# pirovc/ganon

Measured on AMD Instinct MI355X. Metric: Mreads/s classified (150 bp) + IBF-lookup GB/s vs HBM roofline, higher is better.
Workload: dtype u64

## Files before the change

### ganon_amd/csrc/gn_minimiser_lpr.hip

```cpp
#include "gn_internal.h"
#include <type_traits>

#define GN_WAVE 64

namespace
{
struct LprRankLut
{
    uint8_t t[256];
    constexpr LprRankLut() : t{}
    {
        for (int i = 0; i < 256; ++i)
            t[i] = 0;
        t['C'] = t['c'] = 1;
        t['G'] = t['g'] = 2;
        t['T'] = t['t'] = t['U'] = t['u'] = 3;
        t['Y'] = t['y'] = 1;
        t['S'] = t['s'] = 1;
        t['K'] = t['k'] = 2;
        t['B'] = t['b'] = 1;
    }
};
}
__constant__ LprRankLut GN_LPR_RANK_LUT = LprRankLut();

__device__ __forceinline__ uint32_t gn_lpr_wave_max(uint32_t v)
{
#pragma unroll
    for (int off = 32; off >= 1; off >>= 1)
    {
        const uint32_t o = __shfl_xor(v, off);
        v                = o > v ? o : v;
    }
    return v;
}
__device__ __forceinline__ unsigned long long gn_lpr_wave_sum(unsigned long long v)
{
#pragma unroll
    for (int off = 32; off >= 1; off >>= 1)
        v += __shfl_xor(v, off);
    return v;
}

typedef uint32_t gn_u32x4u __attribute__((ext_vector_type(4), aligned(4)));

__global__ __launch_bounds__(64) void gn_minimiser_lpr_kernel(GnMinimiserParams p)
{
    extern __shared__ __attribute__((aligned(16))) uint8_t gn_lpr_smem[];
    const uint32_t lane = threadIdx.x;
    const uint32_t k = p.k, w = p.w;
    const uint32_t K = w - k + 1;
    uint64_t*      bufV = reinterpret_cast<uint64_t*>(gn_lpr_smem);
    uint8_t*       bufP = gn_lpr_smem + (size_t)2 * K * GN_WAVE * 8;
    const uint64_t seed = 0x8F3F73B5CF1C9ADEULL >> (64u - 2u * k);
    const uint64_t mask = k == 32 ? ~0ULL : ((1ULL << (2 * k)) - 1ULL);

    const uint32_t r   = p.read_begin + blockIdx.x * GN_WAVE + lane;
    const bool     inr = r < p.n_reads;
    uint64_t       b1 = 0, len1 = 0, b2 = 0, len2 = 0;
    if (inr)
    {
        b1   = p.off1[r];
        len1 = p.off1[r + 1] - b1;
        if (p.off2)
        {
            b2   = p.off2[r];
            len2 = p.off2[r + 1] - b2;
        }
    }
    const bool too_long = len1 > p.lpr_max_len || len2 > p.lpr_max_len;
    const bool mine     = inr && !too_long;
    if (inr && too_long)
        p.defer_list[atomicAdd(p.defer_count, 1ULL)] = r;

    uint8_t  st = GN_READ_OK;
    uint32_t n  = 0;
    if (mine && len1 < w)
        st = GN_READ_SMALL;
    uint64_t* out = p.hashes + (mine ? p.slot_off[r] : 0);

    for (uint32_t seg = 0; seg < 2; ++seg)
    {
        const uint64_t L64  = seg ? len2 : len1;
        const bool     act  = mine && st == GN_READ_OK && L64 >= w;
        const uint32_t Leff = act ? (uint32_t)L64 : 0u;
        const uint32_t Lmax = gn_lpr_wave_max(Leff);
        if (Lmax == 0)
            continue;
        const uintptr_t  sa  = reinterpret_cast<uintptr_t>(p.bases + (seg ? b2 : b1));
        const uint32_t   o   = (uint32_t)(sa & 3u);
        const uint32_t*  dws = reinterpret_cast<const uint32_t*>(sa & ~(uintptr_t)3);
        const uint32_t   ndw = Leff ? (o + Leff + 3) / 4 : 0;
        auto load4 = [&](uint32_t q) -> gn_u32x4u {
            const uint32_t qc = q < ndw ? q : (ndw ? ndw - 1 : 0u);
            return *reinterpret_cast<const gn_u32x4u*>(dws + qc);
        };
        gn_u32x4u cur4 = load4(0), nxt4 = load4(4);

        uint64_t f = 0, rc = 0;
        uint64_t pre_v = ~0ULL, Wprev = 0;
        uint32_t pre_p = 0, expiry = 0xFFFFFFFFu;
        uint32_t blk = 0, pin = 0;

        auto position = [&](uint32_t i, uint32_t c) {
            const bool on = i < Leff;
            uint64_t   v  = ~0ULL;
            if (on)
            {
                uint64_t       b      = ((c >> 1) ^ (c >> 2)) & 3u;
                const bool     simple = ((0x0030008Au >> (c & 31u)) & 1u) && (c & 0xC0u) == 0x40u;
                if (!simple)
                    b = GN_LPR_RANK_LUT.t[c];
                f                = ((f << 2) | b) & mask;
                rc               = (rc >> 2) | ((3ULL - b) << (2 * (k - 1)));
                const uint64_t x = f ^ seed, y = rc ^ seed;
                v                = x < y ? x : y;
            }
            if (i + 1 < k)
                return;
            const uint32_t pk = i + 1 - k;
            bufV[((size_t)blk * K + pin) * GN_WAVE + lane] = v;
            if (pin == 0 || v <= pre_v)
            {
                pre_v = v;
                pre_p = pk;
            }
            if (pk + 1 >= K)
            {
                const uint32_t j = pk + 1 - K;
                uint64_t       W = pre_v;
                uint32_t       R = pre_p;
                if (pin != K - 1)
                {
                    const size_t   s  = ((size_t)(blk ^ 1u) * K + (pin + 1)) * GN_WAVE + lane;
                    const uint64_t sv = bufV[s];
                    if (sv < pre_v)
                    {
                        W = sv;
                        R = (pk - pin - K) + bufP[s];
                    }
                }
                if (on)
                {
                    const bool emit = j == 0 || j == expiry || v < Wprev;
                    if (emit)
                    {
                        out[n++] = W;
                        expiry   = R + 1u;
                    }
                    Wprev = W;
                }
            }
            if (pin == K - 1)
            {
                uint64_t run_v = ~0ULL;
                uint32_t run_p = K - 1;
                for (int t = (int)K - 1; t >= 0; --t)
                {
                    const size_t   s = ((size_t)blk * K + (uint32_t)t) * GN_WAVE + lane;
                    const uint64_t x = bufV[s];
                    if (x < run_v || t == (int)K - 1)
                    {
                        run_v = x;
                        run_p = (uint32_t)t;
                    }
                    bufV[s] = run_v;
                    bufP[s] = (uint8_t)run_p;
                }
                blk ^= 1u;
                pin = 0;
            }
            else
                ++pin;
        };

        for (uint32_t i0 = 0; i0 < Lmax; i0 += 16)
        {
            const gn_u32x4u nn4 = load4(i0 / 4 + 8);
            uint32_t        d[8] = { cur4.x, cur4.y, cur4.z, cur4.w, nxt4.x, nxt4.y, nxt4.z, nxt4.w };
#pragma unroll
            for (int u = 0; u < 4; ++u)
            {
                const uint64_t win = ((uint64_t)d[u + 1] << 32) | d[u];
#pragma unroll
                for (int t = 0; t < 4; ++t)
                {
                    const uint32_t i = i0 + 4 * u + t;
                    if (i < Lmax)
                        position(i, (uint32_t)(win >> (8u * (o + t))) & 0xFFu);
                }
            }
            cur4 = nxt4;
            nxt4 = nn4;
        }
    }
    unsigned long long mine_total = 0;
    if (mine)
    {
        if (n > 65535u)
            st = GN_READ_BIG;
        else if (st == GN_READ_OK)
            mine_total = n;
        p.n_hashes[r] = n;
        p.status[r]   = st;
    }
    mine_total = gn_lpr_wave_sum(mine_total);
    if (lane == 0 && mine_total)
        atomicAdd(p.total_hashes + (blockIdx.x & 63u), mine_total);
}

#define GN_LPRK_STAGE 24u

template <bool FMIN>
__device__ __forceinline__ uint64_t gn_key_min(uint64_t a, uint64_t b)
{
    if constexpr (FMIN)
    {
        uint64_t r;
        asm("v_min_f64 %0, %1, %2" : "=v"(r) : "v"(a), "v"(b));
        return r;
    }
    else
        return a < b ? a : b;
}

template <int KW, bool FMIN>
__global__ __launch_bounds__(64) void gn_minimiser_lprk_kernel(GnMinimiserParams p)
{
    __shared__ uint64_t stage[GN_LPRK_STAGE * (GN_WAVE + 1)];
    const uint32_t lane = threadIdx.x;
    __shared__ uint8_t rank_lut[256];
#pragma unroll
    for (uint32_t t = 0; t < 4; ++t)
    {
        const uint32_t c   = lane * 4 + t, idx = c & 31u;
        uint32_t       b32 = ((0x0238000Cu >> idx) & 1u) | (((0x00300880u >> idx) & 1u) << 1);
        rank_lut[c]        = (uint8_t)((c & 0xC0u) == 0x40u ? b32 : 0u);
    }
    __builtin_amdgcn_fence(__ATOMIC_RELEASE, "wavefront");
    __builtin_amdgcn_wave_barrier();
    __builtin_amdgcn_fence(__ATOMIC_ACQUIRE, "wavefront");
    const uint32_t k    = p.k;
    const uint64_t seed = 0x8F3F73B5CF1C9ADEULL >> (64u - 2u * k);
    const uint64_t mask = (1ULL << (2 * k)) - 1ULL;
    const uint32_t w    = k + KW - 1;

    const uint32_t r   = p.read_begin + blockIdx.x * GN_WAVE + lane;
    const bool     inr = r < p.n_reads;
    uint64_t       b1 = 0, len1 = 0, b2 = 0, len2 = 0;
    if (inr)
    {
        b1   = p.off1[r];
        len1 = p.off1[r + 1] - b1;
        if (p.off2)
        {
            b2   = p.off2[r];
            len2 = p.off2[r + 1] - b2;
        }
    }
    const bool too_long = len1 > p.lpr_max_len || len2 > p.lpr_max_len;
    const bool mine     = inr && !too_long;
    if (inr && too_long)
        p.defer_list[atomicAdd(p.defer_count, 1ULL)] = r;

    uint8_t  st = GN_READ_OK;
    uint32_t n  = 0;
    if (mine && len1 < w)
        st = GN_READ_SMALL;
    const uint64_t out_base = mine ? p.slot_off[r] : 0;

    for (uint32_t seg = 0; seg < 2; ++seg)
    {
        const uint64_t L64  = seg ? len2 : len1;
        const bool     act  = mine && st == GN_READ_OK && L64 >= w;
        const uint32_t Leff = act ? (uint32_t)L64 : 0u;
        const uint32_t Lmax = gn_lpr_wave_max(Leff);
        if (Lmax == 0)
            continue;
        const uint32_t Lmin = ~gn_lpr_wave_max(~Leff);
        const uint32_t n_seg0 = n;
        const uintptr_t sa  = reinterpret_cast<uintptr_t>(p.bases + (seg ? b2 : b1));
        const uint32_t  o   = (uint32_t)(sa & 3u);
        const uint32_t* dws = reinterpret_cast<const uint32_t*>(sa & ~(uintptr_t)3);
        const uint32_t  ndw = Leff ? (o + Leff + 3) / 4 : 0;
        auto dword_at = [&](uint32_t q) -> uint32_t {
            const uint32_t qc = q < ndw ? q : (ndw ? ndw - 1 : 0u);
            return dws[qc];
        };

        uint64_t       f = 0, rcx = mask;
        const uint64_t seed_rc = seed ^ mask;
        const uint32_t top     = 2 * (k - 1);
        auto roll = [&](uint32_t c) -> uint64_t {
            const uint64_t b = rank_lut[c];
            f                  = ((f << 2) | b) & mask;
            rcx                = (rcx >> 2) | (b << top);
            const uint64_t x = f ^ seed, y = rcx ^ seed_rc;
            return gn_key_min<FMIN>(x, y);
        };
        for (uint32_t q = 0; q * 4 < o + k - 1; ++q)
        {
            const uint32_t dw = dword_at(q);
#pragma unroll
            for (uint32_t t = 0; t < 4; ++t)
            {
                const uint32_t by = q * 4 + t;
                if (by >= o && by - o + 1 < k)
                    (void)roll((dw >> (8u * t)) & 0xFFu);
            }
        }

        uint64_t V[KW], S[KW];
#pragma unroll
        for (int t = 0; t < KW; ++t)
            V[t] = S[t] = ~0ULL;
        uint64_t pre = ~0ULL, Wprev = 0;
        uint32_t expiry = 0xFFFFFFFFu;
        const uint32_t M = Lmax - k + 1;

        constexpr int NDW = (KW + 3) / 4 + 1;
        uint32_t      cur[NDW], nxt[NDW];
        auto fetch = [&](uint32_t blk, uint32_t* dst) {
            const uint32_t q = (o + k - 1 + blk * KW) >> 2;
#pragma unroll
            for (int d = 0; d < NDW; ++d)
                dst[d] = dword_at(q + d);
        };
        fetch(0, cur);
        for (uint32_t blk = 0; blk * KW < M; ++blk)
        {
            fetch(blk + 1, nxt);
            const uint32_t sh = (o + k - 1 + blk * KW) & 3u;
            uint32_t       by[NDW - 1];
#pragma unroll
            for (int d = 0; d + 1 < NDW; ++d)
                by[d] = __builtin_amdgcn_alignbyte(cur[d + 1], cur[d], sh);
            auto block = [&](auto all_on_tag) {
            constexpr bool ALL_ON = decltype(all_on_tag)::value;
#pragma unroll
            for (int pin = 0; pin < KW; ++pin)
            {
                const uint32_t pk = blk * KW + pin;
                const uint32_t i  = pk + k - 1;
                const bool     on = ALL_ON || i < Leff;
                const uint32_t c  = (by[pin >> 2] >> (8 * (pin & 3))) & 0xFFu;
                const uint64_t kv  = (roll(c) << 16) | (uint64_t)(0xFFFFu - pk);
                const uint64_t key = on ? kv : ~0ULL;
                V[pin] = key;
                pre    = pin == 0 ? key : gn_key_min<FMIN>(key, pre);
                if (pk + 1 >= KW)
                {
                    const uint32_t j = pk + 1 - KW;
                    uint64_t       W = pre;
                    if (pin != KW - 1)
                        W = gn_key_min<FMIN>(S[(pin + 1) % KW], pre);
                    if (on)
                    {
                        const bool emit = j == 0 || j == expiry || (key | 0xFFFFull) < (Wprev & ~0xFFFFull);
                        if (emit)
                        {
                            const uint32_t e = n - n_seg0;
                            if (e < GN_LPRK_STAGE)
                                stage[e * (GN_WAVE + 1) + lane] = W >> 16;
                            else
                                p.hashes[out_base + n] = W >> 16;
                            ++n;
                            expiry = (0xFFFFu - (uint32_t)(W & 0xFFFFu)) + 1u;
                        }
                        Wprev = W;
                    }
                }
            }
            };
            if ((blk + 1) * KW + k - 1 <= Lmin)
                block(std::true_type{});
            else
                block(std::false_type{});
            S[KW - 1] = V[KW - 1];
#pragma unroll
            for (int t = KW - 2; t >= 0; --t)
                S[t] = gn_key_min<FMIN>(V[t], S[t + 1]);
#pragma unroll
            for (int d = 0; d < NDW; ++d)
                cur[d] = nxt[d];
        }
        __builtin_amdgcn_fence(__ATOMIC_RELEASE, "wavefront");
        __builtin_amdgcn_wave_barrier();
        __builtin_amdgcn_fence(__ATOMIC_ACQUIRE, "wavefront");
        const uint32_t cnt_mine = act ? (n - n_seg0 < GN_LPRK_STAGE ? n - n_seg0 : GN_LPRK_STAGE) : 0u;
        uint64_t       todo     = __ballot(cnt_mine != 0);
        while (todo)
        {
            const int l = __builtin_ctzll(todo);
            todo &= todo - 1;
            const uint32_t cnt = (uint32_t)__builtin_amdgcn_readlane((int)cnt_mine, l);
            const uint64_t dst0 = out_base + n_seg0;
            const uint64_t dst  = ((uint64_t)(uint32_t)__builtin_amdgcn_readlane((int)(dst0 >> 32), l) << 32) |
                                 (uint32_t)__builtin_amdgcn_readlane((int)(uint32_t)dst0, l);
            if (lane < cnt)
                p.hashes[dst + lane] = stage[lane * (GN_WAVE + 1) + (uint32_t)l];
        }
        __builtin_amdgcn_fence(__ATOMIC_RELEASE, "wavefront");
        __builtin_amdgcn_wave_barrier();
        __builtin_amdgcn_fence(__ATOMIC_ACQUIRE, "wavefront");
    }
    unsigned long long mine_total = 0;
    if (mine)
    {
        if (n > 65535u)
            st = GN_READ_BIG;
        else if (st == GN_READ_OK)
            mine_total = n;
        p.n_hashes[r] = n;
        p.status[r]   = st;
    }
    mine_total = gn_lpr_wave_sum(mine_total);
    if (lane == 0 && mine_total)
        atomicAdd(p.total_hashes + (blockIdx.x & 63u), mine_total);
}

template <int KW>
static void gn_launch_lprk(const GnMinimiserParams& p, hipStream_t st)
{
    const dim3 grid((p.n_reads - p.read_begin + GN_WAVE - 1) / GN_WAVE);
    if (p.k <= 20)
        hipLaunchKernelGGL((gn_minimiser_lprk_kernel<KW, true>), grid, dim3(GN_WAVE), 0, st, p);
    else
        hipLaunchKernelGGL((gn_minimiser_lprk_kernel<KW, false>), grid, dim3(GN_WAVE), 0, st, p);
}

hipError_t gn_launch_minimiser_lpr(const GnMinimiserParams& p, hipStream_t st)
{
    if (p.n_reads <= p.read_begin)
        return hipSuccess;
    const uint32_t K   = p.w - p.k + 1;
    if (K <= 16 && p.k <= 24)
    {
        switch (K)
        {
            case 1: gn_launch_lprk<1>(p, st); break;
            case 2: gn_launch_lprk<2>(p, st); break;
            case 3: gn_launch_lprk<3>(p, st); break;
            case 4: gn_launch_lprk<4>(p, st); break;
            case 5: gn_launch_lprk<5>(p, st); break;
            case 6: gn_launch_lprk<6>(p, st); break;
            case 7: gn_launch_lprk<7>(p, st); break;
            case 8: gn_launch_lprk<8>(p, st); break;
            case 9: gn_launch_lprk<9>(p, st); break;
            case 10: gn_launch_lprk<10>(p, st); break;
            case 11: gn_launch_lprk<11>(p, st); break;
            case 12: gn_launch_lprk<12>(p, st); break;
            case 13: gn_launch_lprk<13>(p, st); break;
            case 14: gn_launch_lprk<14>(p, st); break;
            case 15: gn_launch_lprk<15>(p, st); break;
            default: gn_launch_lprk<16>(p, st); break;
        }
        return hipGetLastError();
    }
    const size_t   lds = (size_t)2 * K * GN_WAVE * 9;
    (void)hipFuncSetAttribute(reinterpret_cast<const void*>(gn_minimiser_lpr_kernel), hipFuncAttributeMaxDynamicSharedMemorySize,
                              (int)lds);
    hipLaunchKernelGGL(gn_minimiser_lpr_kernel, dim3((p.n_reads - p.read_begin + GN_WAVE - 1) / GN_WAVE), dim3(GN_WAVE), lds, st, p);
    return hipGetLastError();
}
```

Baseline: 271.3.

## Split LPR minimiser rolling hash into 32-bit halves and make emission branchless

Rewrites the per-read minimiser kernel so the rolling k-mer state is kept as 32-bit halves, with a 32-bit-only path when k<=16 under FMIN. Emission becomes branchless: every step writes unconditionally into a split 32/16-bit LDS stage, and overflow is handled through a ballot-guarded global store. The kernel also sets waves_per_eu, peels the first block, prefetches ranks in an interleaved way, and flushes two lanes per trip. These changes aim to cut 64-bit ALU work, divergence and register pressure. The cost is extra LDS writes per step and more complex code.

```diff
diff --git a/ganon_amd/csrc/gn_minimiser_lpr.hip b/ganon_amd/csrc/gn_minimiser_lpr.hip
--- a/ganon_amd/csrc/gn_minimiser_lpr.hip
+++ b/ganon_amd/csrc/gn_minimiser_lpr.hip
@@ -210,6 +210,7 @@
 }
 
 #define GN_LPRK_STAGE 24u
+#define GN_LPRK_ROW (GN_WAVE + 1u)
 
 template <bool FMIN>
 __device__ __forceinline__ uint64_t gn_key_min(uint64_t a, uint64_t b)
@@ -224,10 +225,13 @@
         return a < b ? a : b;
 }
 
+__device__ __forceinline__ uint64_t gn_u64_of(uint32_t hi, uint32_t lo) { return ((uint64_t)hi << 32) | lo; }
+
 template <int KW, bool FMIN>
-__global__ __launch_bounds__(64) void gn_minimiser_lprk_kernel(GnMinimiserParams p)
-{
-    __shared__ uint64_t stage[GN_LPRK_STAGE * (GN_WAVE + 1)];
+__global__ __launch_bounds__(64) __attribute__((amdgpu_waves_per_eu(KW <= 13 ? 4 : 3))) void gn_minimiser_lprk_kernel(GnMinimiserParams p)
+{
+    __shared__ uint32_t stage_lo[(GN_LPRK_STAGE + 1u) * GN_LPRK_ROW];
+    __shared__ uint16_t stage_hi[(GN_LPRK_STAGE + 1u) * GN_LPRK_ROW];
     const uint32_t lane = threadIdx.x;
     __shared__ uint8_t rank_lut[256];
 #pragma unroll
@@ -247,16 +251,12 @@
 
     const uint32_t r   = p.read_begin + blockIdx.x * GN_WAVE + lane;
     const bool     inr = r < p.n_reads;
-    uint64_t       b1 = 0, len1 = 0, b2 = 0, len2 = 0;
+    uint64_t       len1 = 0, len2 = 0;
     if (inr)
     {
-        b1   = p.off1[r];
-        len1 = p.off1[r + 1] - b1;
+        len1 = p.off1[r + 1] - p.off1[r];
         if (p.off2)
-        {
-            b2   = p.off2[r];
-            len2 = p.off2[r + 1] - b2;
-        }
+            len2 = p.off2[r + 1] - p.off2[r];
     }
     const bool too_long = len1 > p.lpr_max_len || len2 > p.lpr_max_len;
     const bool mine     = inr && !too_long;
@@ -267,19 +267,20 @@
     uint32_t n  = 0;
     if (mine && len1 < w)
         st = GN_READ_SMALL;
-    const uint64_t out_base = mine ? p.slot_off[r] : 0;
-
-    for (uint32_t seg = 0; seg < 2; ++seg)
-    {
-        const uint64_t L64  = seg ? len2 : len1;
-        const bool     act  = mine && st == GN_READ_OK && L64 >= w;
+
+    auto mate = [&](uint32_t seg, auto tophi_tag) {
+        constexpr bool TOPHI = decltype(tophi_tag)::value;
+        const uint64_t* off = seg ? p.off2 : p.off1;
+        const uint64_t  b0  = mine && off ? off[r] : 0;
+        const uint64_t  L64 = mine && off ? off[r + 1] - b0 : 0;
+        const bool      act = mine && st == GN_READ_OK && L64 >= w;
         const uint32_t Leff = act ? (uint32_t)L64 : 0u;
         const uint32_t Lmax = gn_lpr_wave_max(Leff);
         if (Lmax == 0)
-            continue;
+            return;
         const uint32_t Lmin = ~gn_lpr_wave_max(~Leff);
         const uint32_t n_seg0 = n;
-        const uintptr_t sa  = reinterpret_cast<uintptr_t>(p.bases + (seg ? b2 : b1));
+        const uintptr_t sa  = reinterpret_cast<uintptr_t>(p.bases + b0);
         const uint32_t  o   = (uint32_t)(sa & 3u);
         const uint32_t* dws = reinterpret_cast<const uint32_t*>(sa & ~(uintptr_t)3);
         const uint32_t  ndw = Leff ? (o + Leff + 3) / 4 : 0;
@@ -288,26 +289,59 @@
             return dws[qc];
         };
 
-        uint64_t       f = 0, rcx = mask;
+        uint32_t       f_lo = 0, f_hi = 0, rcx_lo = (uint32_t)mask, rcx_hi = (uint32_t)(mask >> 32);
         const uint64_t seed_rc = seed ^ mask;
-        const uint32_t top     = 2 * (k - 1);
-        auto roll = [&](uint32_t c) -> uint64_t {
-            const uint64_t b = rank_lut[c];
-            f                  = ((f << 2) | b) & mask;
-            rcx                = (rcx >> 2) | (b << top);
-            const uint64_t x = f ^ seed, y = rcx ^ seed_rc;
-            return gn_key_min<FMIN>(x, y);
+        const uint32_t seed_lo = (uint32_t)seed, seed_hi = (uint32_t)(seed >> 32);
+        const uint32_t seed_rc_lo = (uint32_t)seed_rc, seed_rc_hi = (uint32_t)(seed_rc >> 32);
+        const uint32_t mask_lo = (uint32_t)mask, mask_hi = (uint32_t)(mask >> 32);
+        const uint32_t top = (2 * (k - 1)) & 31u;
+        auto rank_of = [&](uint32_t dw, uint32_t t) -> uint32_t { return rank_lut[(dw >> (8u * t)) & 0xFFu]; };
+        auto roll = [&](uint32_t b, uint32_t& v_hi, uint32_t& v_lo) {
+            if constexpr (TOPHI)
+            {
+                f_hi   = __builtin_amdgcn_alignbit(f_hi, f_lo, 30) & mask_hi;
+                f_lo   = (f_lo << 2) | b;
+                rcx_lo = __builtin_amdgcn_alignbit(rcx_hi, rcx_lo, 2);
+                rcx_hi = (rcx_hi >> 2) | (b << top);
+                const uint64_t v = gn_key_min<FMIN>(gn_u64_of(f_hi ^ seed_hi, f_lo ^ seed_lo),
+                                                    gn_u64_of(rcx_hi ^ seed_rc_hi, rcx_lo ^ seed_rc_lo));
+                v_hi = (uint32_t)(v >> 32);
+                v_lo = (uint32_t)v;
+            }
+            else
+            {
+                f_lo   = ((f_lo << 2) | b) & mask_lo;
+                rcx_lo = (rcx_lo >> 2) | (b << top);
+                const uint32_t x = f_lo ^ seed_lo, y = rcx_lo ^ seed_rc_lo;
+                v_hi = 0;
+                v_lo = x < y ? x : y;
+            }
         };
-        for (uint32_t q = 0; q * 4 < o + k - 1; ++q)
         {
-            const uint32_t dw = dword_at(q);
-#pragma unroll
-            for (uint32_t t = 0; t < 4; ++t)
-            {
-                const uint32_t by = q * 4 + t;
-                if (by >= o && by - o + 1 < k)
-                    (void)roll((dw >> (8u * t)) & 0xFFu);
-            }
+            const uint32_t km1 = k - 1;
+            uint32_t       d0 = dword_at(0), d1 = dword_at(1), d2 = dword_at(2), vh, vl, g = 0;
+            for (; 4 * g + 4 <= km1; ++g)
+            {
+                const uint32_t d3 = dword_at(g + 3);
+                const uint32_t dw = __builtin_amdgcn_alignbyte(d1, d0, o);
+                const uint32_t r0 = rank_of(dw, 0), r1 = rank_of(dw, 1), r2 = rank_of(dw, 2), r3 = rank_of(dw, 3);
+                roll(r0, vh, vl);
+                roll(r1, vh, vl);
+                roll(r2, vh, vl);
+                roll(r3, vh, vl);
+                d0 = d1;
+                d1 = d2;
+                d2 = d3;
+            }
+            const uint32_t left = km1 - 4 * g;
+            const uint32_t dw   = __builtin_amdgcn_alignbyte(d1, d0, o);
+            const uint32_t r0 = rank_of(dw, 0), r1 = rank_of(dw, 1), r2 = rank_of(dw, 2);
+            if (left > 0)
+                roll(r0, vh, vl);
+            if (left > 1)
+                roll(r1, vh, vl);
+            if (left > 2)
+                roll(r2, vh, vl);
         }
 
         uint64_t V[KW], S[KW];
@@ -315,10 +349,11 @@
         for (int t = 0; t < KW; ++t)
             V[t] = S[t] = ~0ULL;
         uint64_t pre = ~0ULL, Wprev = 0;
-        uint32_t expiry = 0xFFFFFFFFu;
+        uint32_t expiry_key = 0;
+        uint32_t e = 0;
         const uint32_t M = Lmax - k + 1;
 
-        constexpr int NDW = (KW + 3) / 4 + 1;
+        constexpr int NDW = (KW + 6) / 4;
         uint32_t      cur[NDW], nxt[NDW];
         auto fetch = [&](uint32_t blk, uint32_t* dst) {
             const uint32_t q = (o + k - 1 + blk * KW) >> 2;
@@ -327,14 +362,22 @@
                 dst[d] = dword_at(q + d);
         };
         fetch(0, cur);
-        for (uint32_t blk = 0; blk * KW < M; ++blk)
-        {
+        auto step = [&](uint32_t blk, auto first_tag) {
+            constexpr bool FIRST = decltype(first_tag)::value;
             fetch(blk + 1, nxt);
             const uint32_t sh = (o + k - 1 + blk * KW) & 3u;
-            uint32_t       by[NDW - 1];
-#pragma unroll
-            for (int d = 0; d + 1 < NDW; ++d)
-                by[d] = __builtin_amdgcn_alignbyte(cur[d + 1], cur[d], sh);
+            constexpr int NBY = (KW + 3) / 4;
+            uint32_t      by[NBY], rk[KW];
+#pragma unroll
+            for (int d = 0; d < NBY; ++d)
+                by[d] = __builtin_amdgcn_alignbyte(d + 1 < NDW ? cur[d + 1] : 0u, cur[d], sh);
+            auto ranks = [&](int d) {
+#pragma unroll
+                for (int t = 0; t < 4; ++t)
+                    if (4 * d + t < KW)
+                        rk[4 * d + t] = rank_of(by[d], (uint32_t)t);
+            };
+            ranks(0);
             auto block = [&](auto all_on_tag) {
             constexpr bool ALL_ON = decltype(all_on_tag)::value;
 #pragma unroll
@@ -343,32 +386,38 @@
                 const uint32_t pk = blk * KW + pin;
                 const uint32_t i  = pk + k - 1;
                 const bool     on = ALL_ON || i < Leff;
-                const uint32_t c  = (by[pin >> 2] >> (8 * (pin & 3))) & 0xFFu;
-                const uint64_t kv  = (roll(c) << 16) | (uint64_t)(0xFFFFu - pk);
-                const uint64_t key = on ? kv : ~0ULL;
+                if (pin % 4 == 0 && pin + 4 < KW)
+                {
+                    __builtin_amdgcn_sched_barrier(0);
+                    ranks(pin / 4 + 1);
+                }
+                uint32_t v_hi, v_lo;
+                roll(rk[pin], v_hi, v_lo);
+                const uint32_t kv_hi = TOPHI ? __builtin_amdgcn_alignbit(v_hi, v_lo, 16) : v_lo >> 16;
+                const uint64_t kv    = gn_u64_of(kv_hi, (v_lo << 16) | (0xFFFFu - pk));
+                const uint64_t key   = on ? kv : ~0ULL;
                 V[pin] = key;
                 pre    = pin == 0 ? key : gn_key_min<FMIN>(key, pre);
-                if (pk + 1 >= KW)
+                if (!FIRST || pin == KW - 1)
                 {
                     const uint32_t j = pk + 1 - KW;
                     uint64_t       W = pre;
-                    if (pin != KW - 1)
+                    if (!FIRST && pin != KW - 1)
                         W = gn_key_min<FMIN>(S[(pin + 1) % KW], pre);
-                    if (on)
+                    const bool emit = on && (FIRST || (uint16_t)expiry_key == (uint16_t)(0u - j) || key < (Wprev & ~0xFFFFull));
+                    const uint32_t W_hi = (uint32_t)(W >> 32), W_lo = (uint32_t)W;
+                    const uint32_t h_lo = __builtin_amdgcn_alignbit(W_hi, W_lo, 16);
+                    const uint32_t slot = (e < GN_LPRK_STAGE ? e : GN_LPRK_STAGE) * GN_LPRK_ROW + lane;
+                    stage_lo[slot] = h_lo;
+                    stage_hi[slot] = (uint16_t)(W_hi >> 16);
+                    if (!FIRST && __builtin_expect(__builtin_amdgcn_ballot_w64(emit && e >= GN_LPRK_STAGE) != 0, 0))
                     {
-                        const bool emit = j == 0 || j == expiry || (key | 0xFFFFull) < (Wprev & ~0xFFFFull);
-                        if (emit)
-                        {
-                            const uint32_t e = n - n_seg0;
-                            if (e < GN_LPRK_STAGE)
-                                stage[e * (GN_WAVE + 1) + lane] = W >> 16;
-                            else
-                                p.hashes[out_base + n] = W >> 16;
-                            ++n;
-                            expiry = (0xFFFFu - (uint32_t)(W & 0xFFFFu)) + 1u;
-                        }
-                        Wprev = W;
+                        if (emit && e >= GN_LPRK_STAGE)
+                            p.hashes[p.slot_off[r] + n_seg0 + e] = gn_u64_of(W_hi >> 16, h_lo);
                     }
+                    e += emit ? 1u : 0u;
+                    expiry_key = emit ? W_lo : expiry_key;
+                    Wprev      = W;
                 }
             }
             };
@@ -383,26 +432,40 @@
 #pragma unroll
             for (int d = 0; d < NDW; ++d)
                 cur[d] = nxt[d];
+        };
+        step(0, std::true_type{});
+        for (uint32_t blk = 1; blk * KW < M; ++blk)
+            step(blk, std::false_type{});
+        n = n_seg0 + e;
+        __builtin_amdgcn_fence(__ATOMIC_RELEASE, "wavefront");
+        __builtin_amdgcn_wave_barrier();
+        __builtin_amdgcn_fence(__ATOMIC_ACQUIRE, "wavefront");
+        const uint32_t cnt_mine = e < GN_LPRK_STAGE ? e : GN_LPRK_STAGE;
+        const uint64_t todo     = __ballot(cnt_mine != 0);
+        const uint64_t dst0     = (cnt_mine ? p.slot_off[r] : 0) + n_seg0;
+        const uint32_t slot     = lane & 31u;
+        for (uint32_t trip = 0; trip < GN_WAVE / 2 && (todo >> (2 * trip)) != 0; ++trip)
+        {
+            if (((todo >> (2 * trip)) & 3u) == 0)
+                continue;
+            const int      l   = (int)(2 * trip + (lane >> 5));
+            const uint32_t cnt = (uint32_t)__shfl((int)cnt_mine, l);
+            const uint64_t dst = gn_u64_of((uint32_t)__shfl((int)(dst0 >> 32), l), (uint32_t)__shfl((int)(uint32_t)dst0, l));
+            if (slot < cnt)
+                p.hashes[dst + slot] = gn_u64_of(stage_hi[slot * GN_LPRK_ROW + (uint32_t)l], stage_lo[slot * GN_LPRK_ROW + (uint32_t)l]);
         }
         __builtin_amdgcn_fence(__ATOMIC_RELEASE, "wavefront");
         __builtin_amdgcn_wave_barrier();
         __builtin_amdgcn_fence(__ATOMIC_ACQUIRE, "wavefront");
-        const uint32_t cnt_mine = act ? (n - n_seg0 < GN_LPRK_STAGE ? n - n_seg0 : GN_LPRK_STAGE) : 0u;
-        uint64_t       todo     = __ballot(cnt_mine != 0);
-        while (todo)
-        {
-            const int l = __builtin_ctzll(todo);
-            todo &= todo - 1;
-            const uint32_t cnt = (uint32_t)__builtin_amdgcn_readlane((int)cnt_mine, l);
-            const uint64_t dst0 = out_base + n_seg0;
-            const uint64_t dst  = ((uint64_t)(uint32_t)__builtin_amdgcn_readlane((int)(dst0 >> 32), l) << 32) |
-                                 (uint32_t)__builtin_amdgcn_readlane((int)(uint32_t)dst0, l);
-            if (lane < cnt)
-                p.hashes[dst + lane] = stage[lane * (GN_WAVE + 1) + (uint32_t)l];
-        }
-        __builtin_amdgcn_fence(__ATOMIC_RELEASE, "wavefront");
-        __builtin_amdgcn_wave_barrier();
-        __builtin_amdgcn_fence(__ATOMIC_ACQUIRE, "wavefront");
+    };
+    for (uint32_t seg = 0; seg < 2; ++seg)
+    {
+        if constexpr (!FMIN)
+            mate(seg, std::true_type{});
+        else if (k > 16)
+            mate(seg, std::true_type{});
+        else
+            mate(seg, std::false_type{});
     }
     unsigned long long mine_total = 0;
     if (mine)
```

Result: slower. 267.5 (-1.4%).
